# kkbwilldo/quantizations

Measured on AMD Instinct MI355X. Metric: decode tokens/sec Llama-3-8B NF4 bs=1; 4096×4096 GEMV GB/s vs HBM peak, higher is better.
Workload: dtype f16 activations x 4-bit NF4 weights (exact NF4 codes (fp32 as hi+lo fp16)), fp32 accumulate; 1 GPU; llama3-8b-nf4-dq-decode-bs1; layers=32, prompt_len=32, global_batch=1, stream_batch=1, decode=hipgraph, parallelism=single, projection_groups=64, layer_ops=229, compute_dtype=fp32, rmsnorm_in_grouped_gemv=True, decode_attention=qz_decode_attention, silu_in_gate_up_launch=True, residual_in_gemv_epilogue=True, lm_head=layer_ops.gemv_dense, lm_head_rows_split=False, attention=single GPU

## Files before the change

include/quantizations.h:

```cpp
#ifndef QUANTIZATIONS_H
#define QUANTIZATIONS_H

#ifdef __cplusplus
extern "C" {
#endif

#define QZ_DT_F16 0
#define QZ_DT_BF16 1
#define QZ_DT_F32 2

#define QZ_FP4 0
#define QZ_NF4 1
#define QZ_EXACT_CODES 0x100

#define QZ_OK 0
#define QZ_ERR_ARG (-1)
#define QZ_ERR_BLOCKSIZE (-2)
#define QZ_ERR_SHAPE (-3)
#define QZ_ERR_DTYPE (-4)


int cgemm_4bit_inference_naive_fp32(int m, int n, int k, float *A, unsigned char *B, float *absmax,
                                    float *datatype, float *out, int lda, int ldb, int ldc, int blocksize);

// ... 76 lines not shown
int qz_dequantize_blockwise_8bit(const float *code, const unsigned char *A, const float *absmax, long long n,
                                 int blocksize, const float *offset, float *out, void *stream);

int qz_dequantize_4bit(const unsigned char *A, long long n, int quant_type, int blocksize, const float *absmax,
                       const unsigned char *qabsmax, const float *absmax2, const float *code2, const float *offset,
                       int blocksize2, void *out, int out_dtype, void *stream);

int qz_bench_read_floor(const void *p, long long bytes, unsigned int *sink, void *stream);

int qz_bench_empty(unsigned int *sink, void *stream);

int qz_ipc_handle_size(void);
long long qz_exchange_bytes(int world, long long slot_bytes);
int qz_exchange_alloc(long long bytes, void **ptr);
int qz_exchange_free(void *ptr);
int qz_ipc_get_handle(const void *ptr, void *handle);
int qz_ipc_open_handle(const void *handle, void **ptr);
int qz_ipc_close_handle(void *ptr);
int qz_enable_peer_access(int peer_device);
int qz_allgather_oneshot(const void *src, int nbytes, void *dst, int rank, int world, void *const *peer_bufs,
                         void *own_buf, long long slot_bytes, unsigned int *epoch, unsigned int *status,
                         void *stream);
int qz_allgather_oneshot_mode(const void *src, int nbytes, void *dst, int rank, int world, void *const *peer_bufs,
                              void *own_buf, long long slot_bytes, unsigned int *epoch, unsigned int *status,
                              int mode, void *stream);


int qz_rmsnorm(const void *x, int dtype, long long rows, int K, long long ldx, const void *weight, float eps, void *y,
               long long ldy, void *stream);

int qz_add_rmsnorm(const void *x, const void *residual, int dtype, long long rows, int K, long long ldx,
                   const void *weight, float eps, void *sum, void *y, long long ldy, void *stream);

int qz_rope_qk(int dtype, int B, int S, int D, const void *q, int Hq, const long long *q_str, void *q_out,
               const long long *qo_str, const void *k, int Hk, const long long *k_str, void *k_out,
               const long long *ko_str, const void *cos, const void *sin, const long long *cs_str, void *stream);

int qz_silu_mul(const void *gate, const void *up, int dtype, long long n, void *y, void *stream);


int qz_decode_attention(int dtype, int B, int Hq, int Hkv, int D, int L, const void *q, long long q_row,
                        const void *k, long long k_row, const void *v, long long v_row, const void *cos,
                        const void *sin, long long cs_row, void *k_cache, void *v_cache, const void *mask,
                        long long mask_b, long long mask_j, long long *pos, unsigned int *arrive, void *out,
                        long long out_row, float *work, float scale, void *stream);

long long qz_greedy_step_work_bytes(int B, long long V);
int qz_greedy_step(const void *logits, int dtype, int B, long long V, long long row, long long *hist,
                   long long hist_row, long long hist_len, long long *pos, long long *tok, void *work, void *stream);
int qz_gemv_dense(int M, int K, const void *x, int dtype, const void *W, void *y, void *stream);
int qz_decode_mask(const long long *q_offset, int B, int L, void *mask, void *stream);
int qz_rope_table(int dtype, int B, int S, int D, const long long *pos, long long pos_b, long long pos_s,
                  const void *cos_table, const void *sin_table, long long T, const float *inv_freq, float scale,
                  void *cos, void *sin, void *stream);

int qz_gemv_4bit_pair_silu(const qz_gemv_segment *segs, int K, const void *x, int dtype, int quant_type,
                           int blocksize, int blocksize2, const float *lut, const void *norm_weight, float eps,
                           void *h, void *stream);

#define QZ_LORA_MAX_RANK 64
typedef struct qz_lora_shrink_segment {
  const void *A;
  const float *scaling;
  int r;
  int t_offset;
} qz_lora_shrink_segment;
int qz_lora_shrink(int nseg, const qz_lora_shrink_segment *segs, int K, const void *x, int dtype,
                   const void *norm_weight, float eps, float *t, void *stream);
int qz_gemv_4bit_lora(int M, int K, const void *x, int dtype, const unsigned char *B, int quant_type, int blocksize,
                      const float *absmax, const unsigned char *qabsmax, const float *absmax2, const float *code2,
                      const float *offset, int blocksize2, long long block_base, const float *lut, const void *bias,
                      const void *residual, const void *lora_B, int r, const float *t, void *y, void *stream);
typedef struct qz_lora_segment {
  const void *B;
  int r;
  int t_offset;
} qz_lora_segment;
int qz_gemv_4bit_grouped_lora(int nseg, const qz_gemv_segment *segs, const qz_lora_segment *lora, const float *t,
                              int K, const void *x, int dtype, int quant_type, int blocksize, int blocksize2,
                              const float *lut, const void *norm_weight, float eps, void *stream);

int qz_gemv_knobs(char *buf, int n);
int qz_gemv_set_knob(const char *name, int value);

int qz_version(void);

#ifdef __cplusplus
}
#endif

#endif
```

quantizations_amd/_lib.py:

```python
from __future__ import annotations

import ctypes
import os

import torch

HERE = os.path.dirname(os.path.abspath(__file__))
LIB_PATH = os.environ.get("QZ_LIB_PATH", os.path.join(HERE, "libquantizations.so"))

DT_F16, DT_BF16, DT_F32 = 0, 1, 2
FP4, NF4 = 0, 1
QUANT_TYPES = {"fp4": FP4, "nf4": NF4}
EXACT_CODES = 0x100

_STATUS = {
    -1: "invalid argument (null pointer or negative size)",
    -2: "unsupported blocksize",
    -3: "unsupported shape",
    -4: "unsupported dtype or quant type",
}

_p = ctypes.c_void_p
_i = ctypes.c_int
_ll = ctypes.c_longlong
_f = ctypes.c_float

GEMV_MAX_SEGMENTS = 4
QZ_ERR_SHAPE = -3


class GemvSegment(ctypes.Structure):
    _fields_ = [("M", ctypes.c_int), ("B", ctypes.c_void_p), ("absmax", ctypes.c_void_p),
                ("qabsmax", ctypes.c_void_p), ("absmax2", ctypes.c_void_p), ("code2", ctypes.c_void_p),
                ("offset", ctypes.c_void_p), ("block_base", ctypes.c_longlong), ("bias", ctypes.c_void_p),
                ("y", ctypes.c_void_p)]


class LoraSegment(ctypes.Structure):
    _fields_ = [("B", ctypes.c_void_p), ("r", ctypes.c_int), ("t_offset", ctypes.c_int)]


class LoraShrinkSegment(ctypes.Structure):
    _fields_ = [("A", ctypes.c_void_p), ("scaling", ctypes.c_void_p), ("r", ctypes.c_int),
                ("t_offset", ctypes.c_int)]


LORA_MAX_RANK = 64

SIGNATURES = {
    "cgemm_4bit_inference_naive_fp32": [_i, _i, _i, _p, _p, _p, _p, _p, _i, _i, _i, _i],
    "cquantize_blockwise_fp16_fp4": [_p, _p, _p, _p, _i, _i],
    "cdequantize_blockwise_fp16_fp4": [_p, _p, _p, _p, _i, _i],
    "cquantize_blockwise_fp32": [_p, _p, _p, _p, _i, _i],
    "cdequantize_blockwise_fp32": [_p, _p, _p, _p, _i, _i],
    "cgemm_4bit_inference_naive_fp32_stream": [_i, _i, _i, _p, _p, _p, _p, _p, _i, _i, _i, _i, _p],
    "cquantize_blockwise_fp16_fp4_stream": [_p, _p, _p, _p, _i, _i, _p],
    "cdequantize_blockwise_fp16_fp4_stream": [_p, _p, _p, _p, _i, _i, _p],
    "cquantize_blockwise_fp32_stream": [_p, _p, _p, _p, _i, _i, _p],
    "cdequantize_blockwise_fp32_stream": [_p, _p, _p, _p, _i, _i, _p],
    "qz_gemv_4bit": [_i, _i, _p, _i, _p, _i, _i, _p, _p, _p, _p, _p, _i, _ll, _p, _p, _p, _p],
    "qz_gemv_4bit_residual": [_i, _i, _p, _i, _p, _i, _i, _p, _p, _p, _p, _p, _i, _ll, _p, _p, _p, _p, _p],
    "qz_gemv_4bit_grouped": [_i, _p, _i, _p, _i, _i, _i, _i, _p, _p],
    "qz_gemv_4bit_grouped_rmsnorm": [_i, _p, _i, _p, _i, _i, _i, _i, _p, _p, _f, _p],
    "qz_gemv_4bit_pair_silu": [_p, _i, _p, _i, _i, _i, _i, _p, _p, _f, _p, _p],
    "qz_lora_shrink": [_i, _p, _i, _p, _i, _p, _f, _p, _p],
    "qz_gemv_4bit_lora": [_i, _i, _p, _i, _p, _i, _i, _p, _p, _p, _p, _p, _i, _ll, _p, _p, _p, _p, _i, _p, _p, _p],
    "qz_gemv_4bit_grouped_lora": [_i, _p, _p, _p, _i, _p, _i, _i, _i, _i, _p, _p, _f, _p],
    "qz_decode_attention": [_i, _i, _i, _i, _i, _i, _p, _ll, _p, _ll, _p, _ll, _p, _p, _ll, _p, _p, _p, _ll, _ll,
                            _p, _p, _p, _ll, _p, _f, _p],
    "qz_gemm_4bit": [_i, _i, _i, _p, _i, _i, _p, _i, _i, _p, _p, _p, _p, _p, _i, _p, _p, _i, _p, _ll, _p],
    "qz_gemm_4bit_workspace_size": [_i, _i, _i],
    "qz_gemm_16bit": [_i, _i, _i, _p, _i, _i, _p, _p, _p, _i, _p],
    "qz_gemm_16bit_ok": [_i, _i, _i, _p, _i, _p, _p, _i],
    "qz_gemm_4bit_grouped": [_i, _p, _i, _i, _p, _i, _i, _i, _i, _i, _p],
    "qz_quantize_4bit": [_p, _i, _ll, _i, _i, _p, _p, _p],
    "qz_absmax_mean_workspace": [_ll],
    "qz_absmax_mean": [_p, _ll, _p, _p, _p],
    "qz_quantize_blockwise_8bit": [_p, _p, _ll, _i, _p, _p, _p, _p],
    "qz_dequantize_blockwise_8bit": [_p, _p, _p, _ll, _i, _p, _p, _p],
    "qz_dequantize_4bit": [_p, _ll, _i, _i, _p, _p, _p, _p, _p, _i, _p, _i, _p],
    "qz_rmsnorm": [_p, _i, _ll, _i, _ll, _p, _f, _p, _ll, _p],
    "qz_rope_qk": [_i, _i, _i, _i, _p, _i, _p, _p, _p, _p, _i, _p, _p, _p, _p, _p, _p, _p],
    "qz_silu_mul": [_p, _p, _i, _ll, _p, _p],
    "qz_decode_mask": [_p, _i, _i, _p, _p],
    "qz_gemv_dense": [_i, _i, _p, _i, _p, _p, _p],
    "qz_greedy_step": [_p, _i, _i, _ll, _ll, _p, _ll, _ll, _p, _p, _p, _p],
    "qz_greedy_step_work_bytes": [_i, _ll],
    "qz_rope_table": [_i, _i, _i, _i, _p, _ll, _ll, _p, _p, _ll, _p, _f, _p, _p, _p],
    "qz_add_rmsnorm": [_p, _p, _i, _ll, _i, _ll, _p, _f, _p, _p, _ll, _p],
    "qz_bench_read_floor": [_p, _ll, _p, _p],
    "qz_bench_empty": [_p, _p],
    "qz_ipc_handle_size": [],
    "qz_exchange_bytes": [_i, _ll],
    "qz_exchange_alloc": [_ll, _p],
    "qz_exchange_free": [_p],
    "qz_ipc_get_handle": [_p, _p],
    "qz_ipc_open_handle": [_p, _p],
    "qz_ipc_close_handle": [_p],
    "qz_enable_peer_access": [_i],
    "qz_allgather_oneshot": [_p, _i, _p, _i, _i, _p, _p, _ll, _p, _p, _p],
    "qz_allgather_oneshot_mode": [_p, _i, _p, _i, _i, _p, _p, _ll, _p, _p, _i, _p],
    "qz_gemv_knobs": [_p, _i],
    "qz_gemv_set_knob": [ctypes.c_char_p, _i],
    "qz_version": [],
}
RESTYPES = {"qz_absmax_mean_workspace": _ll, "qz_gemm_4bit_workspace_size": _ll, "qz_exchange_bytes": _ll,
            "qz_greedy_step_work_bytes": _ll}


def _load():
    if not os.path.exists(LIB_PATH):
        raise ImportError(
            f"libquantizations.so not found at {LIB_PATH}: build it with "
            "`python -c 'import __graft_entry__ as g; g.build()'` (hipcc --offload-arch=gfx950)")
    lib = ctypes.CDLL(LIB_PATH)
    for name, args in SIGNATURES.items():
        fn = getattr(lib, name)
        fn.argtypes = args
        fn.restype = RESTYPES.get(name, _i)
    return lib


lib = _load()


class QuantizationsError(RuntimeError):
    pass


def check(rc: int, what: str) -> None:
    if rc != 0:
        msg = _STATUS.get(rc, f"HIP error {rc}")
        raise QuantizationsError(f"{what} failed: {msg}")


def dtype_code(dt: torch.dtype) -> int:
    if dt == torch.float16:
        return DT_F16
    if dt == torch.bfloat16:
        return DT_BF16
    if dt == torch.float32:
        return DT_F32
    raise NotImplementedError(f"dtype {dt} is not supported by the 4-bit kernels")


def stream_of(t: torch.Tensor) -> int:
    return torch.cuda.current_stream(t.device).cuda_stream


def ptr(t) -> int:
    return 0 if t is None else t.data_ptr()


def gemv_knobs() -> dict:
    import json
    buf = ctypes.create_string_buffer(512)
    n = lib.qz_gemv_knobs(buf, len(buf))
    return json.loads(buf.value.decode()) if 0 < n < len(buf) else {}


def set_gemv_knob(name: str, value: int) -> None:
    check(lib.qz_gemv_set_knob(name.encode(), int(value)), f"qz_gemv_set_knob({name})")
```

quantizations_amd/csrc/gemv.hip:

```cpp
#include "gemv_core.h"

namespace qz {

static int env_int(const char *name, int dflt) {
  const char *e = getenv(name);
  return e && *e ? atoi(e) : dflt;
}
static Knobs read_knobs() {
  Knobs k;
  k.wide8 = env_int("QZ_GEMV_WIDE8", 1) != 0;
  const int nr = env_int("QZ_GROUPED_NORM_R", 0);
  k.norm_r = (nr == 1 || nr == 2 || nr == 4) ? nr : 0;
  const int pr = env_int("QZ_PAIR_R", 0);
  k.pair_r = (pr == 2 || pr == 3 || pr == 4 || pr == 6 || pr == 8) ? pr : 0;
  k.pair_wt = env_int("QZ_PAIR_WT", 1) != 0;
  k.pair_ps = env_int("QZ_PAIR_PS", -1);
  k.pair_wk1 = env_int("QZ_PAIR_WK1", 2);
  return k;
}
static Knobs g_knobs = read_knobs();
Knobs &gemv_knobs() { return g_knobs; }
static int g_gemm16_sched = env_int("QZ_GEMM16_SCHED", 971);
int &gemm16_sched() { return g_gemm16_sched; }

template <bool DQ, int DT, int R, int WK, int NW, bool FS, bool CL, bool WT, bool TWO, int STAMP = 0>
__global__ __launch_bounds__(NW * 64) void k_gemv_4bit(GemvParams p) {
  gemv_body<DQ, DT, R, WK, NW, FS, CL, WT, false, false, TWO, false, STAMP>(p, blockIdx.x);
}

template <bool DQ, int DT, int R, int WK, bool FS, bool CL, bool NRM, bool TWO>
__global__ __launch_bounds__(256) void k_gemv_4bit_grouped(GemvGroup g) {
  const int b = blockIdx.x;
  int s = 0;
#pragma unroll
  for (int i = 1; i < kMaxSeg; ++i)
    if (i < g.nseg && b >= g.start[i]) s = i;
  s = __builtin_amdgcn_readfirstlane(s);
  const GemvParams seg = g.seg[s];
  const int start = g.start[s];
  gemv_body<DQ, DT, R, WK, 4, FS, CL, false, NRM, false, TWO, false>(seg, b - start);
}

template <bool DQ, int DT, int R, bool CL, bool NRM, bool TWO, bool PS = false, bool WT = false>
__global__ __launch_bounds__(256) void k_gemv_4bit_pair(GemvGroup g) {
  const int wave = __builtin_amdgcn_readfirstlane((int)threadIdx.x / kWave);
  const GemvParams seg = g.seg[wave >> 1];
  gemv_body<DQ, DT, R, 1, 4, true, CL, WT, NRM, true, TWO, PS>(seg, blockIdx.x, g.seg);
}

template <bool DQ, int DT>
__global__ __launch_bounds__(256) void k_gemv_4bit_generic(GemvParams p, int quant_type) {
  gemv_generic_body<DQ, DT>(p, quant_type);
}


template <bool DQ, int DT, bool FS, bool CL>
static void launch_vec(const GemvParams &p, int R, int WK, hipStream_t s) {
  const int RG = 4 / WK;
  const unsigned grid = (unsigned)((p.M + R * RG - 1) / (R * RG));
#define QZ_GV(RR, WW, TWO_) \
  hipLaunchKernelGGL((k_gemv_4bit<DQ, DT, RR, WW, 4, FS, CL, false, (WW == 1 && TWO_)>), dim3(grid), dim3(256), 0, s, p)
#define QZ_GV_RW(TWO_)                        \
  do {                                        \
    if (R == 4 && WK == 2) QZ_GV(4, 2, TWO_); \
    else if (R == 4) QZ_GV(4, 1, TWO_);       \
    else if (R == 2) QZ_GV(2, 1, TWO_);       \
    else if (WK == 1) QZ_GV(1, 1, TWO_);      \
    else if (WK == 2) QZ_GV(1, 2, TWO_);      \
    else QZ_GV(1, 4, TWO_);                   \
  } while (0)
  if constexpr (FS) {
    if (two_steps(p.K, WK, true)) { QZ_GV_RW(true); return; }
  }
  if constexpr (FS && CL && DT == QZ_DT_F16) {
    if (WK == 1 && (R == 2 || R == 4) && p.K >= 14336 && gemv_knobs().wide8) {
      const unsigned g8 = (unsigned)((p.M + R * 8 - 1) / (R * 8));
      if (R == 4) hipLaunchKernelGGL((k_gemv_4bit<DQ, DT, 4, 1, 8, FS, CL, true, false>), dim3(g8), dim3(512), 0, s, p);
      else hipLaunchKernelGGL((k_gemv_4bit<DQ, DT, 2, 1, 8, FS, CL, true, false>), dim3(g8), dim3(512), 0, s, p);
      return;
    }
  }
  QZ_GV_RW(false);
#undef QZ_GV_RW
#undef QZ_GV
}

template <bool DQ, bool FS, bool CL>
static int dispatch_dt(const GemvParams &p, int dtype, int R, int WK, hipStream_t s) {
  switch (dtype) {
    case QZ_DT_F16: launch_vec<DQ, QZ_DT_F16, FS, CL>(p, R, WK, s); return QZ_OK;
    case QZ_DT_BF16:
      if constexpr (!CL) { launch_vec<DQ, QZ_DT_BF16, FS, false>(p, R, WK, s); return QZ_OK; }
      break;
    case QZ_DT_F32:
      if constexpr (!CL) { launch_vec<DQ, QZ_DT_F32, FS, false>(p, R, WK, s); return QZ_OK; }
      break;
  }
// ... 97 lines not shown
      if (!full_steps(K, blocksize, blocksize2, dq, segs[i].block_base)) return QZ_ERR_SHAPE;
      g.seg[i].nw = nw;
      g.seg[i].eps = eps;
    }
  }
  if (!all_vec || total_m > INT32_MAX) {
    for (int i = 0; i < nseg; ++i) {
      const qz_gemv_segment &q = segs[i];
      const int rc = qz_gemv_4bit(q.M, K, x, dtype, q.B, quant_type, blocksize, q.absmax, q.qabsmax, q.absmax2,
                                  q.code2, q.offset, blocksize2, q.block_base, lut, q.bias, q.y, stream);
      if (rc != QZ_OK) return rc;
    }
    return QZ_OK;
  }
  int R, WK;
  choose_geometry((int)total_m, K, dtype, &R, &WK);
  if (nw && gemv_knobs().norm_r && WK == 1) R = gemv_knobs().norm_r;
  const int rows_per_block = R * (4 / WK);
  int blocks = 0;
  for (int i = 0; i < nseg; ++i) {
    set_tables(quant_type & ~QZ_EXACT_CODES, lut, cl, dtype, &g.seg[i]);
    g.start[i] = blocks;
    blocks += (g.seg[i].M + rows_per_block - 1) / rows_per_block;
  }
  for (int i = nseg; i < kMaxSeg; ++i) g.start[i] = blocks;
  g.total = blocks;
  if (nw && blocks > kNormMaxBlocks) return QZ_ERR_SHAPE;
  if (nw && WK != 1 && (long long)blocks * K > kNormSplitMaxValues) return QZ_ERR_SHAPE;
  bool all_fs = true;
  for (int i = 0; i < nseg; ++i) all_fs = all_fs && full_steps(K, blocksize, blocksize2, dq, segs[i].block_base);
  hipStream_t s = (hipStream_t)stream;
  const bool two = two_steps(K, WK, all_fs || nw);
  const size_t lds = nw ? (size_t)K * 2 : 0;
#define QZ_GR1(DQ_, DT_, RR, WW, FS_, CL_, NRM_)                                                            \
  do {                                                                                                    \
    if (FS_ && two && WW == 1)                                                                            \
      hipLaunchKernelGGL((k_gemv_4bit_grouped<DQ_, DT_, RR, WW, FS_, CL_, NRM_, (FS_ && WW == 1)>), dim3(blocks), \
                         dim3(256), lds, s, g);                                                           \
    else hipLaunchKernelGGL((k_gemv_4bit_grouped<DQ_, DT_, RR, WW, FS_, CL_, NRM_, false>), dim3(blocks),      \
                            dim3(256), lds, s, g);                                                        \
  } while (0)
#define QZ_GR_RW(DQ_, DT_, FS_, CL_, NRM_)                                                                  \
  do {                                                                                                    \
    if (R == 4 && WK == 2) QZ_GR1(DQ_, DT_, 4, 2, FS_, CL_, NRM_);                                        \
    else if (R == 4) QZ_GR1(DQ_, DT_, 4, 1, FS_, CL_, NRM_);                                              \
    else if (R == 2) QZ_GR1(DQ_, DT_, 2, 1, FS_, CL_, NRM_);                                              \
    else if (WK == 1) QZ_GR1(DQ_, DT_, 1, 1, FS_, CL_, NRM_);                                             \
    else if (WK == 2) QZ_GR1(DQ_, DT_, 1, 2, FS_, CL_, NRM_);                                             \
    else QZ_GR1(DQ_, DT_, 1, 4, FS_, CL_, NRM_);                                                          \
  } while (0)
#define QZ_GR_DT(DQ_, FS_)                                                                                  \
  do {                                                                                                    \
    if (dtype == QZ_DT_F16) { if (cl) QZ_GR_RW(DQ_, QZ_DT_F16, FS_, true, false); else QZ_GR_RW(DQ_, QZ_DT_F16, FS_, false, false); } \
    else if (dtype == QZ_DT_BF16) QZ_GR_RW(DQ_, QZ_DT_BF16, FS_, false, false);                         \
    else QZ_GR_RW(DQ_, QZ_DT_F32, FS_, false, false);                                                    \
  } while (0)
  if (nw) {
    if (dtype == QZ_DT_F16) {
      if (dq) { if (cl) QZ_GR_RW(true, QZ_DT_F16, true, true, true); else QZ_GR_RW(true, QZ_DT_F16, true, false, true); }
      else { if (cl) QZ_GR_RW(false, QZ_DT_F16, true, true, true); else QZ_GR_RW(false, QZ_DT_F16, true, false, true); }
    } else {
      if (dq) QZ_GR_RW(true, QZ_DT_BF16, true, false, true); else QZ_GR_RW(false, QZ_DT_BF16, true, false, true);
    }
  } else if (all_fs) { if (dq) QZ_GR_DT(true, true); else QZ_GR_DT(false, true); }
  else { if (dq) QZ_GR_DT(true, false); else QZ_GR_DT(false, false); }
#undef QZ_GR_DT
#undef QZ_GR_RW
#undef QZ_GR1
  QZ_LAUNCH_CHECK();
  return QZ_OK;
}

extern "C" int qz_gemv_4bit_grouped(int nseg, const qz_gemv_segment *segs, int K, const void *x, int dtype,
                                    int quant_type, int blocksize, int blocksize2, const float *lut, void *stream) {
  return gemv_grouped_impl(nseg, segs, K, x, dtype, quant_type, blocksize, blocksize2, lut, nullptr, 0.0f, stream);
}

extern "C" int qz_gemv_4bit_grouped_rmsnorm(int nseg, const qz_gemv_segment *segs, int K, const void *x, int dtype,
                                            int quant_type, int blocksize, int blocksize2, const float *lut,
                                            const void *norm_weight, float eps, void *stream) {
  if (!norm_weight || !x) return QZ_ERR_ARG;
  return gemv_grouped_impl(nseg, segs, K, x, dtype, quant_type, blocksize, blocksize2, lut, norm_weight, eps, stream);
}

template <bool DQ, int DT, int R, bool CL, bool NRM>
static void launch_pair_wt(unsigned grid, size_t lds, hipStream_t s, const GemvGroup &g, bool two) {
  if constexpr (CL && NRM && DT == QZ_DT_F16 && (R == 2 || R == 4)) {
    if (two) hipLaunchKernelGGL((k_gemv_4bit_pair<DQ, DT, R, CL, NRM, true, true, true>), dim3(grid), dim3(256), lds, s, g);
    else hipLaunchKernelGGL((k_gemv_4bit_pair<DQ, DT, R, CL, NRM, false, true, true>), dim3(grid), dim3(256), lds, s, g);
  }
}

template <bool DQ, int DT, int R, bool CL, bool NRM>
static void launch_pair_ps_loop(unsigned grid, int blocks, size_t lds, hipStream_t s, const GemvGroup &g) {
  if constexpr (NRM)
    hipLaunchKernelGGL((k_gemv_4bit_pair<DQ, DT, R, CL, NRM, false, true>), dim3(grid), dim3(256), lds, s, g);
  else
    hipLaunchKernelGGL((k_gemv_4bit_pair<DQ, DT, R, CL, NRM, false>), dim3(blocks), dim3(256), lds, s, g);
}

extern "C" int qz_gemv_4bit_pair_silu(const qz_gemv_segment *segs, int K, const void *x, int dtype, int quant_type,
                                      int blocksize, int blocksize2, const float *lut, const void *norm_weight,
                                      float eps, void *h, void *stream) {
  if (!segs || !h || !x) return QZ_ERR_ARG;
  if (segs[0].M != segs[1].M) return QZ_ERR_SHAPE;
  if (dtype != QZ_DT_F16 && dtype != QZ_DT_BF16) return QZ_ERR_SHAPE;
  GemvGroup g;
  g.nseg = 2;
  const bool cl = exact_codes(quant_type, lut) && dtype == QZ_DT_F16;
  const bool dq = segs[0].qabsmax != nullptr;
  for (int i = 0; i < 2; ++i) {
    const qz_gemv_segment &q = segs[i];
    bool v;
    const int st = make_params(q.M, K, x, dtype, q.B, quant_type, blocksize, q.absmax, q.qabsmax, q.absmax2, q.code2,
                               q.offset, blocksize2, q.block_base, lut, q.bias, h, &g.seg[i], &v);
    if (st != QZ_OK) return st;
    if ((q.qabsmax != nullptr) != dq || !v || !full_steps(K, blocksize, blocksize2, dq, q.block_base))
      return QZ_ERR_SHAPE;
    set_tables(quant_type & ~QZ_EXACT_CODES, lut, cl, dtype, &g.seg[i]);
    g.seg[i].nw = norm_weight;
    g.seg[i].eps = eps;
  }
  const int M = segs[0].M;
  if (M == 0) return QZ_OK;
  if (norm_weight && (K % 8 != 0 || K > 16384 || ((uintptr_t)x | (uintptr_t)norm_weight) % 16 != 0))
    return QZ_ERR_SHAPE;
  int R, WK;
  choose_geometry(2 * M, K, dtype, &R, &WK);
  if (WK != 1) {
    const int wk1 = gemv_knobs().pair_wk1;
    if (wk1 == 0 || (norm_weight && wk1 != 2)) return QZ_ERR_SHAPE;
    WK = 1;
  }
  if (gemv_knobs().pair_r) R = gemv_knobs().pair_r;
  const int blocks = (M + 2 * R - 1) / (2 * R);
  if (norm_weight && blocks > kNormMaxBlocks) return QZ_ERR_SHAPE;
  for (int i = 2; i < kMaxSeg; ++i) g.start[i] = 0;
  hipStream_t s = (hipStream_t)stream;
  const size_t lds = norm_weight ? (size_t)K * 2 : 0;
  const bool two = two_steps(K, 1, true);
  const int cus = device_cus();
  const size_t img = norm_weight ? (size_t)K * 2 : 0;
  const int per_cu_wt = (int)std::min<size_t>(3, kLdsPerCU / (2 * kTabDwords * 4 + img + 4096));
  const int per_cu = (int)std::min<size_t>(3, kLdsPerCU / (kTabDwords * 4 + img + 4096));
  const bool wt_ok = cl && norm_weight && (R == 2 || R == 4) && blocks >= 3 * 2 * cus && per_cu_wt >= 2 &&
                     gemv_knobs().pair_wt;
  int pgrid_i = 0;
  if (gemv_knobs().pair_ps >= 0) {
    const int ps = gemv_knobs().pair_ps;
    pgrid_i = ps <= 0 ? 0 : ps <= 8 ? cus * ps : ps;
  } else if (norm_weight) {
    pgrid_i = (wt_ok ? 2 : per_cu) * cus;
  }
  const unsigned pgrid = (unsigned)max(pgrid_i, 1);
  const bool persist = pgrid_i > 0 && pgrid_i < blocks;
  const bool pair_wt = persist && wt_ok;
#define QZ_PS(DQ_, DT_, RR, CL_, NRM_)                                                                               \
  do {                                                                                                              \
    if (pair_wt) launch_pair_wt<DQ_, DT_, RR, CL_, NRM_>(pgrid, lds, s, g, two);                                        \
    else if (persist && two) hipLaunchKernelGGL((k_gemv_4bit_pair<DQ_, DT_, RR, CL_, NRM_, true, true>), dim3(pgrid), \
                                                dim3(256), lds, s, g);                                              \
    else if (persist) launch_pair_ps_loop<DQ_, DT_, RR, CL_, NRM_>(pgrid, blocks, lds, s, g);                      \
    else if (two) hipLaunchKernelGGL((k_gemv_4bit_pair<DQ_, DT_, RR, CL_, NRM_, true>), dim3(blocks), dim3(256),    \
                                     lds, s, g);                                                                    \
    else hipLaunchKernelGGL((k_gemv_4bit_pair<DQ_, DT_, RR, CL_, NRM_, false>), dim3(blocks), dim3(256), lds, s, g); \
  } while (0)
#define QZ_PS_R(DQ_, DT_, CL_, NRM_)                  \
  do {                                                \
    if (R == 4) QZ_PS(DQ_, DT_, 4, CL_, NRM_);        \
    else if (R == 8) QZ_PS(DQ_, DT_, 8, CL_, NRM_);   \
    else if (R == 6) QZ_PS(DQ_, DT_, 6, CL_, NRM_);   \
    else if (R == 3) QZ_PS(DQ_, DT_, 3, CL_, NRM_);   \
    else if (R == 1) QZ_PS(DQ_, DT_, 1, CL_, NRM_);   \
    else QZ_PS(DQ_, DT_, 2, CL_, NRM_);               \
  } while (0)
#define QZ_PS_N(DQ_, DT_, CL_)                                                         \
  do {                                                                                 \
    if (norm_weight) QZ_PS_R(DQ_, DT_, CL_, true); else QZ_PS_R(DQ_, DT_, CL_, false); \
  } while (0)
  if (dtype == QZ_DT_F16) {
    if (dq) { if (cl) QZ_PS_N(true, QZ_DT_F16, true); else QZ_PS_N(true, QZ_DT_F16, false); }
    else { if (cl) QZ_PS_N(false, QZ_DT_F16, true); else QZ_PS_N(false, QZ_DT_F16, false); }
  } else {
    if (dq) QZ_PS_N(true, QZ_DT_BF16, false); else QZ_PS_N(false, QZ_DT_BF16, false);
  }
#undef QZ_PS_N
#undef QZ_PS_R
#undef QZ_PS
  QZ_LAUNCH_CHECK();
  return QZ_OK;
}

extern "C" int qz_gemv_knobs(char *buf, int n) {
  char tmp[320];
  const int len = snprintf(tmp, sizeof(tmp),
                           "{\"QZ_GEMV_WIDE8\": %d, \"QZ_GROUPED_NORM_R\": %d, \"QZ_PAIR_R\": %d, \"QZ_PAIR_WT\": %d, "
                           "\"QZ_PAIR_PS\": %d, \"QZ_PAIR_WK1\": %d, \"QZ_GEMM16_SCHED\": %d, \"cus\": %d}",
                           gemv_knobs().wide8, gemv_knobs().norm_r, gemv_knobs().pair_r, gemv_knobs().pair_wt,
                           gemv_knobs().pair_ps, gemv_knobs().pair_wk1, gemm16_sched(), device_cus());
  if (buf && n > len) memcpy(buf, tmp, (size_t)len + 1);
  return len;
}

extern "C" int qz_gemv_set_knob(const char *name, int value) {
  if (!name) return QZ_ERR_ARG;
  Knobs &k = gemv_knobs();
  if (!strcmp(name, "QZ_GEMV_WIDE8")) k.wide8 = value != 0;
  else if (!strcmp(name, "QZ_GROUPED_NORM_R")) k.norm_r = (value == 1 || value == 2 || value == 4) ? value : 0;
  else if (!strcmp(name, "QZ_PAIR_R")) k.pair_r = (value == 2 || value == 3 || value == 4 || value == 6 || value == 8) ? value : 0;
  else if (!strcmp(name, "QZ_PAIR_WT")) k.pair_wt = value != 0;
  else if (!strcmp(name, "QZ_PAIR_PS")) k.pair_ps = value;
  else if (!strcmp(name, "QZ_PAIR_WK1")) k.pair_wk1 = value;
  else if (!strcmp(name, "QZ_GEMM16_SCHED")) gemm16_sched() = value;
  else return QZ_ERR_ARG;
  return QZ_OK;
}
```

quantizations_amd/csrc/gemv_core.h:

```cpp
#pragma once
#include "common.h"

#include <atomic>
#include <cstdio>
#include <cstdlib>
#include <cstring>

namespace qz {

constexpr int kTabCopies = 32;
constexpr int kTabDwords = 256 * kTabCopies;
constexpr int kTabCopiesCL = 16;

constexpr uint16_t f16_bits_rne_c(float f) {
  const uint32_t u = __builtin_bit_cast(uint32_t, f);
  const uint32_t sign = (u >> 16) & 0x8000u, au = u & 0x7FFFFFFFu;
  if (au == 0) return (uint16_t)sign;
  const uint32_t e = (au >> 23) - 127u + 15u, m = au & 0x7FFFFFu;
  uint32_t h = (e << 10) | (m >> 13);
  const uint32_t rem = m & 0x1FFFu;
  if (rem > 0x1000u || (rem == 0x1000u && (h & 1u))) h += 1u;
  return (uint16_t)(sign | h);
}
struct ByteTable {
// ... 12 lines not shown
                                0.7229568362236023f, 1.0f};
constexpr ByteTable make_nf4_table() {
  uint16_t c[16] = {};
  for (int i = 0; i < 16; ++i) c[i] = f16_bits_rne_c(kNF4Host[i]);
  return make_byte_table(c);
}
constexpr uint16_t kFP4x12Bits[16] = {0x0000, 0x2C00, 0x4800, 0x4A00, 0x4400, 0x4600, 0x4000, 0x4200,
                                      0x8000, 0xAC00, 0xC800, 0xCA00, 0xC400, 0xC600, 0xC000, 0xC200};
constexpr int kNF4ExactShift = 14;
constexpr float f16_value_c(uint16_t h) {
  const float sgn = (h & 0x8000u) ? -1.0f : 1.0f;
  const int e = (h >> 10) & 31;
  if (e == 0) return sgn * 0.0f;
  float v = 1.0f + (float)(h & 0x3FFu) / 1024.0f;
  for (int i = 15; i < e; ++i) v *= 2.0f;
  for (int i = e; i < 15; ++i) v *= 0.5f;
  return sgn * v;
}
constexpr ByteTable make_nf4_exact_table() {
  uint16_t hi[16] = {}, lo[16] = {};
  for (int i = 0; i < 16; ++i) {
    const float c = kNF4Host[i] * (float)(1 << kNF4ExactShift);
    hi[i] = f16_bits_rne_c(c);
    lo[i] = f16_bits_rne_c(c - f16_value_c(hi[i]));
  }
  ByteTable t{};
  for (int e = 0; e < 256; ++e) {
    const uint32_t h = (uint32_t)hi[e >> 4] | ((uint32_t)hi[e & 15] << 16);
    const uint32_t l = (uint32_t)lo[e >> 4] | ((uint32_t)lo[e & 15] << 16);
    t.v[4 * e + 0] = h; t.v[4 * e + 1] = l; t.v[4 * e + 2] = h; t.v[4 * e + 3] = l;
  }
  return t;
}
constexpr uint16_t bf16_bits_rne_c(float f) {
  const uint32_t u = __builtin_bit_cast(uint32_t, f);
  return (uint16_t)((u + 0x7FFFu + ((u >> 16) & 1u)) >> 16);
}
constexpr float bf16_value_c(uint16_t b) { return __builtin_bit_cast(float, (uint32_t)b << 16); }
constexpr ByteTable make_bf16_table(const float (&c)[16]) {
  uint16_t hi[16] = {}, lo[16] = {};
  for (int i = 0; i < 16; ++i) {
    hi[i] = bf16_bits_rne_c(c[i]);
    lo[i] = bf16_bits_rne_c(c[i] - bf16_value_c(hi[i]));
  }
  ByteTable t{};
  for (int e = 0; e < 256; ++e) {
    const uint32_t h = (uint32_t)hi[e >> 4] | ((uint32_t)hi[e & 15] << 16);
    const uint32_t l = (uint32_t)lo[e >> 4] | ((uint32_t)lo[e & 15] << 16);
    t.v[4 * e + 0] = h; t.v[4 * e + 1] = l; t.v[4 * e + 2] = h; t.v[4 * e + 3] = l;
  }
  return t;
}
constexpr float kFP4x12Host[16] = {0.0f, 0.0625f, 8.0f, 12.0f, 4.0f, 6.0f, 2.0f, 3.0f,
                                   -0.0f, -0.0625f, -8.0f, -12.0f, -4.0f, -6.0f, -2.0f, -3.0f};
constexpr ByteTable make_f32_table(const float (&c)[16]) {
  ByteTable t{};
  for (int e = 0; e < 256; ++e) {
    const uint32_t a = __builtin_bit_cast(uint32_t, c[e >> 4]), b = __builtin_bit_cast(uint32_t, c[e & 15]);
    t.v[4 * e + 0] = a; t.v[4 * e + 1] = b; t.v[4 * e + 2] = a; t.v[4 * e + 3] = b;
  }
  return t;
}
static __device__ const ByteTable g_byte_tab_nf4 = make_nf4_table();
static __device__ const ByteTable g_byte_tab_nf4x = make_nf4_exact_table();
static __device__ const ByteTable g_byte_tab_fp4 = make_byte_table(kFP4x12Bits);
static __device__ const ByteTable g_byte_tab_nf4_bf = make_bf16_table(kNF4Host);
static __device__ const ByteTable g_byte_tab_fp4_bf = make_bf16_table(kFP4x12Host);
static __device__ const ByteTable g_byte_tab_nf4_f32 = make_f32_table(kNF4Host);
static __device__ const ByteTable g_byte_tab_fp4_f32 = make_f32_table(kFP4x12Host);
static_assert(bf16_bits_rne_c(0.07958029955625534f) == 0x3DA3, "bf16 RNE of an NF4 code");
static_assert(f16_bits_rne_c(0.07958029955625534f) == 0x2D18, "fp16 RNE of an NF4 code");

typedef uint32_t u32x4 __attribute__((ext_vector_type(4)));
typedef uint32_t u32x2 __attribute__((ext_vector_type(2)));
typedef __bf16 bf16x2_t __attribute__((ext_vector_type(2)));

template <int DT> __device__ __forceinline__ float round_store(float v) {
  if constexpr (DT == QZ_DT_F16) return __half2float(__ushort_as_half(f32_to_f16_bits(v)));
  else if constexpr (DT == QZ_DT_BF16) return __bfloat162float(__float2bfloat16(v));
  else return v;
}
template <int DT> __device__ __forceinline__ float add_res(float o, const void *res, long long row) {
  return res ? __fadd_rn(load_f32<DT>(res, row), round_store<DT>(o)) : o;
}

template <int DT> __device__ __forceinline__ uint32_t pack16(float a, float b) {
  if constexpr (DT == QZ_DT_F16) {
    return (uint32_t)f32_to_f16_bits(a) | ((uint32_t)f32_to_f16_bits(b) << 16);
  } else {
    return (uint32_t)__builtin_bit_cast(uint16_t, __float2bfloat16(a)) |
           ((uint32_t)__builtin_bit_cast(uint16_t, __float2bfloat16(b)) << 16);
  }
}

struct GemvParams {
  const unsigned char *B;
  const void *x;
  ScaleSrc sc;
  const void *bias;
  void *y;
  const float *lut;
  long long block_base;
  int M, K;
  int bs_log2, bs2_log2;
  float out_scale;
  int tabsel;
  const void *nw;
  float eps;
  const void *res;
};

struct LoraOp {
  const void *B;
  const float *t;
  int r;
};

__device__ __forceinline__ float dot2(uint32_t a, uint32_t b, float c) {
  return __builtin_amdgcn_fdot2(__builtin_bit_cast(h2_t, a), __builtin_bit_cast(h2_t, b), c, false);
}

template <typename T> __device__ __forceinline__ T keep_s(T v) {
  asm volatile("" : "+s"(v));
  return v;
}
template <typename T> __device__ __forceinline__ T *keep_sp(T *v) {
  typedef __attribute__((address_space(1))) T *gptr;
  gptr g = (gptr)v;
  asm volatile("" : "+s"(g));
  return (T *)g;
}

#ifdef QZ_STAMPS
__device__ unsigned long long *g_qz_stamp;
#define QZ_STAMP_DECL unsigned long long qz_st_[6] = {0, 0, 0, 0, 0, 0}
#define QZ_STAMP(k)                                                                  \
  do {                                                                               \
    if constexpr ((STAMP & 3) != 0 && ((STAMP & 3) == 1 || (k) == 0 || (k) == 4)) {  \
      __builtin_amdgcn_sched_barrier(0);                                             \
      asm volatile("s_memrealtime %0\n\ts_waitcnt lgkmcnt(0)" : "=s"(qz_st_[k])::"memory"); \
      __builtin_amdgcn_sched_barrier(0);                                             \
    }                                                                                \
  } while (0)
#define QZ_STAMP_FLUSH(wave_id)                                                      \
  do {                                                                               \
    if constexpr ((STAMP & 3) != 0) {                                                \
      uint32_t xcc, hw;                                                              \
      asm volatile("s_getreg_b32 %0, hwreg(HW_REG_XCC_ID)" : "=s"(xcc));             \
      asm volatile("s_getreg_b32 %0, hwreg(HW_REG_HW_ID)" : "=s"(hw));               \
      qz_st_[5] = ((unsigned long long)xcc << 32) | hw;                              \
      if ((threadIdx.x & 63) == 0) {                                                 \
        if constexpr ((STAMP & 3) == 2) {                                            \
          g_qz_stamp[(size_t)(wave_id) * 8 + 0] = qz_st_[0];                         \
          g_qz_stamp[(size_t)(wave_id) * 8 + 4] = qz_st_[4];                         \
        } else {                                                                     \
          for (int k_ = 0; k_ < 6; ++k_) g_qz_stamp[(size_t)(wave_id) * 8 + k_] = qz_st_[k_]; \
        }                                                                            \
      }                                                                              \
    }                                                                                \
  } while (0)
#else
#define QZ_STAMP_DECL
#define QZ_STAMP(k) do {} while (0)
#define QZ_STAMP_FLUSH(wave_id) do {} while (0)
#endif

// ... 271 lines not shown
__device__ __forceinline__ uint32_t norm_x_off(uint32_t chunk) {
  const uint32_t s = chunk >> 8, l = (chunk >> 2) & 63u, i = chunk & 3u;
  return (s << 12) + (l << 6) + ((i ^ ((l >> 2) & 3u)) << 4);
}

constexpr int kMaxSeg = 4;
struct GemvGroup {
  GemvParams seg[kMaxSeg];
  int start[kMaxSeg];
  int nseg;
  int total;
};
struct LoraGroup {
  LoraOp seg[kMaxSeg];
};

template <bool DQ, int DT, int R, int WK, int NW, bool FS, bool CL, bool WT, bool NRM, bool PAIR, bool TWO, bool PS,
          int STAMP = 0, bool LORA = false>
__device__ __forceinline__ void gemv_body(const GemvParams &p_in, const int block, const GemvParams *pair = nullptr,
                                          const LoraOp *lora = nullptr) {
  static_assert(!LORA || (!PAIR && DT != QZ_DT_F32), "adapter operand: single / grouped launches, 16-bit activations");
  static_assert(!NRM || (NW == 4 && FS && DT != QZ_DT_F32), "fused pre-norm: 4 waves, full steps, 16-bit activations");
  static_assert(!PAIR || (NW == 4 && WK == 1 && DT != QZ_DT_F32), "pair: 4 waves, WK = 1, 16-bit activations");
  static_assert(!PS || (PAIR && FS), "persistent form: pair launches, full steps");
  static_assert(!TWO || (FS && WK == 1), "two-step form: full steps, whole rows per wave");
  static_assert(!CL || DT == QZ_DT_F16, "exact codes are the fp16-activation table");
  static_assert(NW * 64 >= 256, "one byte-table entry per thread");
  constexpr int kPieces = WT ? 16 : kTabCopies / 4;
  QZ_STAMP_DECL;
  QZ_STAMP(0);
  const GemvParams p = load_params(p_in);
  constexpr int RG = NW / WK;
  constexpr bool kBF = DT == QZ_DT_BF16;
  constexpr bool kF32 = DT == QZ_DT_F32;
  constexpr bool kWide = CL || kBF || kF32;
  __shared__ float s_code2[PAIR ? 2 : 1][DQ ? 256 : 1];
  __shared__ float s_part[NW][R];
  __shared__ float s_part2[PS ? 2 : 1][NW][R];
  __shared__ __attribute__((aligned(16))) uint32_t s_tab[(WT ? 2 : 1) * kTabDwords];
  extern __shared__ __attribute__((aligned(16))) unsigned char s_x[];

  const int lane = threadIdx.x & (kWave - 1);
  const int wave = __builtin_amdgcn_readfirstlane(threadIdx.x / kWave);
  const int wk = wave % WK;
  const int rg = wave / WK;
  int row0 = PAIR ? (block * 2 + (wave & 1)) * R : (block * RG + rg) * R;
  const int cb = PAIR ? (wave >> 1) : 0;
  const int row_bytes = p.K >> 1;
  const int nsteps = (row_bytes + 1023) >> 10;

  float c2 = 0.0f, c2b = 0.0f, offset = 0.0f;
  if constexpr (DQ) {
    if constexpr (PAIR) {
      c2 = keep_sp(pair[0].sc.code2)[threadIdx.x];
      c2b = keep_sp(pair[1].sc.code2)[threadIdx.x];
    } else if (NW * 64 == 256 || threadIdx.x < 256) {
      c2 = p.sc.code2[threadIdx.x & 255];
    }
    offset = *p.sc.offset;
  }
  u32x4 tab_entry = {0u, 0u, 0u, 0u};
  if (!p.lut && threadIdx.x < 256) {
    const ByteTable *bt = kF32 ? (p.tabsel ? &g_byte_tab_fp4_f32 : &g_byte_tab_nf4_f32)
                          : kBF ? (p.tabsel ? &g_byte_tab_fp4_bf : &g_byte_tab_nf4_bf)
                                : (CL ? &g_byte_tab_nf4x : (p.tabsel ? &g_byte_tab_fp4 : &g_byte_tab_nf4));
    tab_entry = reinterpret_cast<const u32x4 *>(bt->v)[threadIdx.x];
  }
  constexpr int kNChunks = NRM ? 8 : 1;
  constexpr int kNHeld = NRM ? 2 : 1;
  u32x4 nx[kNChunks], nwh[kNHeld];
  const int n_nchunk = p.K >> 3;
  if constexpr (NRM) {
#pragma unroll
    for (int i = 0; i < kNChunks; ++i) {
      const int c = (int)threadIdx.x + 256 * i;
      if (c < n_nchunk) nx[i] = reinterpret_cast<const u32x4 *>(p.x)[c];
    }
#pragma unroll
    for (int i = 0; i < kNHeld; ++i) {
      const int c = (int)threadIdx.x + 256 * i;
      if (c < n_nchunk) nwh[i] = reinterpret_cast<const u32x4 *>(p.nw)[c];
    }
    __builtin_amdgcn_sched_barrier(0);
  }
  typedef StepLoads<DQ, DT, R, NRM, FS> Loads;
  Loads cur, other;
  int s = wk;
  cur.issue(p, row0, s < nsteps ? s : 0, lane, row_bytes);
  float lo_b[LORA ? R : 1], lo_t = 0.0f;
  bool lo_on = false;
  if constexpr (LORA) {
    const int lr = keep_s(lora->r);
    const char *lB = reinterpret_cast<const char *>(keep_sp(lora->B));
    const float *lt = keep_sp(lora->t);
    lo_on = lane < lr && wk == 0;
    const int j = lo_on ? lane : 0;
    lo_t = lt[j];
#pragma unroll
    for (int r = 0; r < R; ++r) {
      const size_t row = (size_t)min(row0 + r, p.M - 1);
      lo_b[r] = load_f32<DT>(lB + row * (size_t)lr * 2u, j);
    }
  }
  const bool have = s < nsteps;
  const int n_my = have ? (nsteps - wk + WK - 1) / WK : 0;
  if constexpr (DQ) {
    if (NW * 64 == 256 || threadIdx.x < 256) s_code2[0][threadIdx.x & 255] = c2;
    if constexpr (PAIR) s_code2[PAIR ? 1 : 0][threadIdx.x] = c2b;
  }
  __shared__ float s_nss[NRM ? 4 : 1];
  if constexpr (NRM) {
    float ss = 0.0f;
#pragma unroll
    for (int i = 0; i < kNChunks; ++i)
      if ((int)threadIdx.x + 256 * i < n_nchunk) ss = norm_chunk_ss<DT>(nx[i], ss);
    ss = norm_wave_sum(ss);
    if (lane == 0) s_nss[wave] = ss;
  }
  float out_scale = p.out_scale;
  if constexpr (kF32) {
    if (p.lut) {
      out_scale = 1.0f;
      build_byte_table_f32<NW * 64, kPieces>(s_tab, p.lut);
    } else if (threadIdx.x < 256) {
      store_byte_table_entry<kPieces>(s_tab, tab_entry);
    }
  } else if constexpr (kBF) {
    if (p.lut) {
      out_scale = 1.0f;
      build_byte_table_bf16<NW * 64, kPieces>(s_tab, p.lut);
    } else if (threadIdx.x < 256) {
      store_byte_table_entry<kPieces>(s_tab, tab_entry);
    }
  } else if constexpr (CL) {
    if (p.lut) {
      const int S = lut_shift(p.lut);
      out_scale = ldexpf(1.0f, -S);
      build_byte_table_exact<NW * 64, kPieces>(s_tab, p.lut, S);
    } else if (threadIdx.x < 256 && (STAMP & 48) == 0) {
      store_byte_table_entry<kPieces>(s_tab, tab_entry);
    }
  } else if (threadIdx.x < 256) {
    store_byte_table_entry<kPieces>(s_tab, tab_entry);
  }
  if constexpr ((STAMP & 32) == 0) __syncthreads();
  if constexpr (NRM) {
    const float tot = __fadd_rn(__fadd_rn(s_nss[0], s_nss[1]), __fadd_rn(s_nss[2], s_nss[3]));
    const float rs = rsqrtf(__fadd_rn(__fmul_rn(tot, 1.0f / (float)p.K), p.eps));
#pragma unroll
    for (int i = 0; i < kNChunks; ++i) {
      const int c = (int)threadIdx.x + 256 * i;
      if (c < n_nchunk) {
        const u32x4 xv = i < kNHeld ? nx[i] : reinterpret_cast<const u32x4 *>(p.x)[c];
        const u32x4 wv = i < kNHeld ? nwh[i < kNHeld ? i : 0] : reinterpret_cast<const u32x4 *>(p.nw)[c];
        *reinterpret_cast<u32x4 *>(s_x + norm_x_off((uint32_t)c)) = norm_chunk_apply<DT>(xv, wv, rs);
      }
    }
    __syncthreads();
  }
  QZ_STAMP(1);
  const uint32_t jb = WT ? (kWide ? (uint32_t)(lane & 31) << 3 : (uint32_t)lane << 2)
                        : (kWide ? (uint32_t)(lane & (kTabCopiesCL - 1)) << 3 : (uint32_t)(lane & 31) << 2);

  float acc[R];
#pragma unroll
  for (int r = 0; r < R; ++r) acc[r] = 0.0f;
// ... 81 lines not shown
        } else {
          consume(cur);
        }
      }
      const int nb = blk + (int)gridDim.x;
      if (nb >= nblocks) {
        pair_out(blk, it & 1);
        break;
      }
      const int nrow0 = (nb * 2 + (wave & 1)) * R;
      cur.issue(p, nrow0, s, lane, row_bytes);
      __builtin_amdgcn_sched_barrier(0);
      pair_out(blk, it & 1);
#pragma unroll
      for (int r = 0; r < R; ++r) acc[r] = 0.0f;
      blk = nb;
      row0 = nrow0;
    }
    return;
  } else if constexpr (TWO) {
    other.issue(p, row0, s + WK, lane, row_bytes);
    __builtin_amdgcn_sched_barrier(0);
    consume(cur);
    QZ_STAMP(2);
    consume(other);
  } else if (have) {
    const int n = n_my;
    int j = 0;
    for (; j + 2 < n; j += 2) {
      other.issue(p, row0, s + WK, lane, row_bytes);
      __builtin_amdgcn_sched_barrier(0);
      consume(cur);
      cur.issue(p, row0, s + 2 * WK, lane, row_bytes);
      __builtin_amdgcn_sched_barrier(0);
      consume(other);
      s += 2 * WK;
    }
    if (n - j == 2) {
      other.issue(p, row0, s + WK, lane, row_bytes);
      __builtin_amdgcn_sched_barrier(0);
      consume(cur);
      QZ_STAMP(2);
      consume(other);
    } else {
      consume(cur);
    }
  }

  if constexpr (LORA) {
    const float inv = __fdiv_rn(1.0f, out_scale);
#pragma unroll
    for (int r = 0; r < R; ++r) acc[r] = lo_on ? fmaf(__fmul_rn(lo_b[r], lo_t), inv, acc[r]) : acc[r];
  }
  QZ_STAMP(3);
  if constexpr (PAIR) {
    float v[R];
#pragma unroll
    for (int r = 0; r < R; ++r) v[r] = wave_sum_last(acc[r]);
    if (lane == kWave - 1) {
#pragma unroll
      for (int r = 0; r < R; ++r) {
        float o = v[r] * out_scale;
        if (p.bias) o += load_f32<DT>(p.bias, min(row0 + r, p.M - 1));
        s_part[wave][r] = o;
      }
    }
    __syncthreads();
    if ((int)threadIdx.x < 2 * R) {
      const int g2 = threadIdx.x / R, r = threadIdx.x % R;
      const int row = (block * 2 + g2) * R + r;
      if (row < p.M) {
        const float gv = round_store<DT>(s_part[g2][r]), uv = round_store<DT>(s_part[2 + g2][r]);
        const float a = round_store<DT>(__fdiv_rn(gv, __fadd_rn(1.0f, expf(-gv))));
        store_f32<DT>(keep_sp(pair[0].y), row, __fmul_rn(a, uv));
      }
    }
    return;
  }
  if constexpr (WK == 1) {
    float v[R];
#pragma unroll
    for (int r = 0; r < R; ++r) v[r] = wave_sum_last(acc[r]);
    if (lane == kWave - 1) {
      constexpr bool kPack = DT != QZ_DT_F32 && R % 2 == 0;
      const bool pack = kPack && row0 + R <= p.M && (reinterpret_cast<uintptr_t>(p.y) & 3u) == 0;
      if (pack) {
#pragma unroll
        for (int r = 0; r < R; r += 2) {
          float o0 = v[r] * out_scale, o1 = v[r + 1] * out_scale;
          if (p.bias) {
            o0 += load_f32<DT>(p.bias, row0 + r);
            o1 += load_f32<DT>(p.bias, row0 + r + 1);
          }
          o0 = add_res<DT>(o0, p.res, row0 + r);
          o1 = add_res<DT>(o1, p.res, row0 + r + 1);
          reinterpret_cast<uint32_t *>(p.y)[(row0 + r) >> 1] = pack16<DT>(o0, o1);
        }
      } else {
#pragma unroll
        for (int r = 0; r < R; ++r) {
          const int row = row0 + r;
          if (row < p.M) {
            float o = v[r] * out_scale;
            if (p.bias) o += load_f32<DT>(p.bias, row);
            o = add_res<DT>(o, p.res, row);
            store_f32<DT>(p.y, row, o);
          }
        }
      }
    }
    QZ_STAMP(4);
    QZ_STAMP_FLUSH(block * NW + wave);
    return;
  }
#pragma unroll
  for (int r = 0; r < R; ++r) {
    const float v = wave_sum_last(acc[r]);
    if (lane == kWave - 1) s_part[wave][r] = v;
  }
  __syncthreads();
  if ((int)threadIdx.x < RG * R) {
    const int g = threadIdx.x / R, r = threadIdx.x % R;
    const int row = (block * RG + g) * R + r;
    if (row < p.M) {
      float v = 0.0f;
#pragma unroll
      for (int k = 0; k < WK; ++k) v += s_part[g * WK + k][r];
      v *= out_scale;
      if (p.bias) v += load_f32<DT>(p.bias, row);
      store_f32<DT>(p.y, row, add_res<DT>(v, p.res, row));
    }
  }
}

template <bool DQ, int DT, bool LORA = false>
__device__ __forceinline__ void gemv_generic_body(const GemvParams &p, int quant_type, const LoraOp *lora = nullptr) {
  __shared__ float s_lut[16];
  if (threadIdx.x < 16) s_lut[threadIdx.x] = p.lut ? p.lut[threadIdx.x] : 0.0f;
  __syncthreads();
  const int lane = threadIdx.x & (kWave - 1);
  const int row = blockIdx.x * 4 + threadIdx.x / kWave;
  if (row >= p.M) return;
  const float offset = DQ ? *p.sc.offset : 0.0f;
  float acc = 0.0f;
  for (int k = lane; k < p.K; k += kWave) {
    const long long e = (long long)row * p.K + k;
    const uint32_t byte = p.B[e >> 1];
    const uint32_t nib = (e & 1) ? (byte & 0xFu) : (byte >> 4);
    const long long b = p.block_base + (e >> p.bs_log2);
    float am;
    if constexpr (DQ) am = __fadd_rn(__fmul_rn(p.sc.code2[p.sc.qabsmax[b]], p.sc.absmax2[b >> p.bs2_log2]), offset);
    else am = p.sc.absmax[b];
    float c;
    if (p.lut) c = s_lut[nib];
    else if (quant_type == QZ_NF4) c = kNF4[nib];
    else c = (nib & 8u ? -1.0f : 1.0f) * dequant_fp4_tree(nib & 7u, 1.0f);
    acc = fmaf(load_f32<DT>(p.x, k), __fmul_rn(c, am), acc);
  }
  if constexpr (LORA) {
    if (lane < lora->r) acc = fmaf(load_f32<DT>(lora->B, (long long)row * lora->r + lane), lora->t[lane], acc);
  }
  acc = wave_sum_last(acc);
  if (lane == kWave - 1) {
    if (p.bias) acc += load_f32<DT>(p.bias, row);
    store_f32<DT>(p.y, row, add_res<DT>(acc, p.res, row));
  }
}


struct Knobs {
  int wide8;
  int norm_r;
  int pair_r;
  int pair_wt;
  int pair_ps;
  int pair_wk1;
};
constexpr int kNormMaxBlocks = 4096;
constexpr long long kNormSplitMaxValues = 1LL << 23;
constexpr size_t kLdsPerCU = 160 * 1024;
Knobs &gemv_knobs();

static int ilog2(long long v) {
  int l = 0;
  while ((1LL << l) < v) ++l;
  return (1LL << l) == v ? l : -1;
}

// ... 74 lines not shown
```

Measured before the change: 553.2 tokens/s.

## Prefetch residual/bias in GEMV prologue and base pair persistence on geometry

For non-pair, single-split, 4-wave GEMV kernels, the residual and bias values are now loaded into registers before the main loop instead of in the epilogue, which hides their load latency behind weight streaming. The pair (gate/up + SiLU) launcher now decides whether the wide-table persistent path applies using the default-R block count and the actual persistent grid size rather than a fixed 2×CUs. It also allows R=1 as a pair knob and records the last pair launch geometry for inspection. Holding the extra per-row values in registers may raise register pressure, and loads are issued for all lanes rather than only the storing lane.

```diff
diff --git a/include/quantizations.h b/include/quantizations.h
--- a/include/quantizations.h
+++ b/include/quantizations.h
@@ -182,6 +182,7 @@
 
 int qz_gemv_knobs(char *buf, int n);
 int qz_gemv_set_knob(const char *name, int value);
+int qz_gemv_pair_last_geometry(int *out);
 
 int qz_version(void);
 
diff --git a/quantizations_amd/_lib.py b/quantizations_amd/_lib.py
--- a/quantizations_amd/_lib.py
+++ b/quantizations_amd/_lib.py
@@ -102,6 +102,7 @@
     "qz_allgather_oneshot_mode": [_p, _i, _p, _i, _i, _p, _p, _ll, _p, _p, _i, _p],
     "qz_gemv_knobs": [_p, _i],
     "qz_gemv_set_knob": [ctypes.c_char_p, _i],
+    "qz_gemv_pair_last_geometry": [_p],
     "qz_version": [],
 }
 RESTYPES = {"qz_absmax_mean_workspace": _ll, "qz_gemm_4bit_workspace_size": _ll, "qz_exchange_bytes": _ll,
@@ -159,5 +160,11 @@
     return json.loads(buf.value.decode()) if 0 < n < len(buf) else {}
 
 
+def pair_last_geometry() -> dict:
+    out = (ctypes.c_int * 4)()
+    check(lib.qz_gemv_pair_last_geometry(ctypes.cast(out, ctypes.c_void_p)), "qz_gemv_pair_last_geometry")
+    return {"R": out[0], "grid": out[1], "blocks": out[2], "wide_table": bool(out[3])}
+
+
 def set_gemv_knob(name: str, value: int) -> None:
     check(lib.qz_gemv_set_knob(name.encode(), int(value)), f"qz_gemv_set_knob({name})")
diff --git a/quantizations_amd/csrc/gemv.hip b/quantizations_amd/csrc/gemv.hip
--- a/quantizations_amd/csrc/gemv.hip
+++ b/quantizations_amd/csrc/gemv.hip
@@ -6,13 +6,14 @@
   const char *e = getenv(name);
   return e && *e ? atoi(e) : dflt;
 }
+static bool pair_r_ok(int r) { return r == 1 || r == 2 || r == 3 || r == 4 || r == 6 || r == 8; }
 static Knobs read_knobs() {
   Knobs k;
   k.wide8 = env_int("QZ_GEMV_WIDE8", 1) != 0;
   const int nr = env_int("QZ_GROUPED_NORM_R", 0);
   k.norm_r = (nr == 1 || nr == 2 || nr == 4) ? nr : 0;
   const int pr = env_int("QZ_PAIR_R", 0);
-  k.pair_r = (pr == 2 || pr == 3 || pr == 4 || pr == 6 || pr == 8) ? pr : 0;
+  k.pair_r = pair_r_ok(pr) ? pr : 0;
   k.pair_wt = env_int("QZ_PAIR_WT", 1) != 0;
   k.pair_ps = env_int("QZ_PAIR_PS", -1);
   k.pair_wk1 = env_int("QZ_PAIR_WK1", 2);
@@ -276,6 +277,8 @@
   if (!norm_weight || !x) return QZ_ERR_ARG;
   return gemv_grouped_impl(nseg, segs, K, x, dtype, quant_type, blocksize, blocksize2, lut, norm_weight, eps, stream);
 }
+
+static int g_pair_last[4] = {0, 0, 0, 0};
 
 template <bool DQ, int DT, int R, bool CL, bool NRM>
 static void launch_pair_wt(unsigned grid, size_t lds, hipStream_t s, const GemvGroup &g, bool two) {
@@ -326,6 +329,7 @@
     if (wk1 == 0 || (norm_weight && wk1 != 2)) return QZ_ERR_SHAPE;
     WK = 1;
   }
+  const int blocks_geom = (M + 2 * R - 1) / (2 * R);
   if (gemv_knobs().pair_r) R = gemv_knobs().pair_r;
   const int blocks = (M + 2 * R - 1) / (2 * R);
   if (norm_weight && blocks > kNormMaxBlocks) return QZ_ERR_SHAPE;
@@ -337,18 +341,21 @@
   const size_t img = norm_weight ? (size_t)K * 2 : 0;
   const int per_cu_wt = (int)std::min<size_t>(3, kLdsPerCU / (2 * kTabDwords * 4 + img + 4096));
   const int per_cu = (int)std::min<size_t>(3, kLdsPerCU / (kTabDwords * 4 + img + 4096));
-  const bool wt_ok = cl && norm_weight && (R == 2 || R == 4) && blocks >= 3 * 2 * cus && per_cu_wt >= 2 &&
-                     gemv_knobs().pair_wt;
+  const int ps_knob = gemv_knobs().pair_ps;
+  const int knob_grid = ps_knob <= 0 ? 0 : ps_knob <= 8 ? cus * ps_knob : ps_knob;
+  const int wt_grid = ps_knob >= 0 ? knob_grid : 2 * cus;
+  const bool wt_ok = cl && norm_weight && (R == 2 || R == 4) && blocks_geom >= 3 * wt_grid &&
+                     per_cu_wt >= 2 && gemv_knobs().pair_wt;
   int pgrid_i = 0;
-  if (gemv_knobs().pair_ps >= 0) {
-    const int ps = gemv_knobs().pair_ps;
-    pgrid_i = ps <= 0 ? 0 : ps <= 8 ? cus * ps : ps;
-  } else if (norm_weight) {
-    pgrid_i = (wt_ok ? 2 : per_cu) * cus;
-  }
+  if (ps_knob >= 0) pgrid_i = knob_grid;
+  else if (norm_weight) pgrid_i = (wt_ok ? 2 : per_cu) * cus;
   const unsigned pgrid = (unsigned)max(pgrid_i, 1);
   const bool persist = pgrid_i > 0 && pgrid_i < blocks;
   const bool pair_wt = persist && wt_ok;
+  g_pair_last[0] = R;
+  g_pair_last[1] = persist ? pgrid_i : blocks;
+  g_pair_last[2] = blocks;
+  g_pair_last[3] = pair_wt;
 #define QZ_PS(DQ_, DT_, RR, CL_, NRM_)                                                                               \
   do {                                                                                                              \
     if (pair_wt) launch_pair_wt<DQ_, DT_, RR, CL_, NRM_>(pgrid, lds, s, g, two);                                        \
@@ -385,6 +392,12 @@
   return QZ_OK;
 }
 
+extern "C" int qz_gemv_pair_last_geometry(int *out) {
+  if (!out) return QZ_ERR_ARG;
+  memcpy(out, g_pair_last, sizeof(g_pair_last));
+  return QZ_OK;
+}
+
 extern "C" int qz_gemv_knobs(char *buf, int n) {
   char tmp[320];
   const int len = snprintf(tmp, sizeof(tmp),
@@ -401,7 +414,7 @@
   Knobs &k = gemv_knobs();
   if (!strcmp(name, "QZ_GEMV_WIDE8")) k.wide8 = value != 0;
   else if (!strcmp(name, "QZ_GROUPED_NORM_R")) k.norm_r = (value == 1 || value == 2 || value == 4) ? value : 0;
-  else if (!strcmp(name, "QZ_PAIR_R")) k.pair_r = (value == 2 || value == 3 || value == 4 || value == 6 || value == 8) ? value : 0;
+  else if (!strcmp(name, "QZ_PAIR_R")) k.pair_r = pair_r_ok(value) ? value : 0;
   else if (!strcmp(name, "QZ_PAIR_WT")) k.pair_wt = value != 0;
   else if (!strcmp(name, "QZ_PAIR_PS")) k.pair_ps = value;
   else if (!strcmp(name, "QZ_PAIR_WK1")) k.pair_wk1 = value;
diff --git a/quantizations_amd/csrc/gemv_core.h b/quantizations_amd/csrc/gemv_core.h
--- a/quantizations_amd/csrc/gemv_core.h
+++ b/quantizations_amd/csrc/gemv_core.h
@@ -118,6 +118,9 @@
 }
 template <int DT> __device__ __forceinline__ float add_res(float o, const void *res, long long row) {
   return res ? __fadd_rn(load_f32<DT>(res, row), round_store<DT>(o)) : o;
+}
+template <int DT> __device__ __forceinline__ float add_res_value(float o, bool has_res, float res) {
+  return has_res ? __fadd_rn(res, round_store<DT>(o)) : o;
 }
 
 template <int DT> __device__ __forceinline__ uint32_t pack16(float a, float b) {
@@ -555,6 +558,20 @@
       if (c < n_nchunk) nwh[i] = reinterpret_cast<const u32x4 *>(p.nw)[c];
     }
     __builtin_amdgcn_sched_barrier(0);
+  }
+  constexpr bool kEarlyEp = !PAIR && WK == 1 && NW == 4;
+  float ep_res[R], ep_bias[R];
+  if constexpr (kEarlyEp) {
+#pragma unroll
+    for (int r = 0; r < R; ++r) ep_res[r] = ep_bias[r] = 0.0f;
+    if (p.res) {
+#pragma unroll
+      for (int r = 0; r < R; ++r) ep_res[r] = load_f32<DT>(p.res, min(row0 + r, p.M - 1));
+    }
+    if (p.bias) {
+#pragma unroll
+      for (int r = 0; r < R; ++r) ep_bias[r] = load_f32<DT>(p.bias, min(row0 + r, p.M - 1));
+    }
   }
   typedef StepLoads<DQ, DT, R, NRM, FS> Loads;
   Loads cur, other;
@@ -802,6 +819,14 @@
 #pragma unroll
     for (int r = 0; r < R; ++r) v[r] = wave_sum_last(acc[r]);
     if (lane == kWave - 1) {
+      auto bias_of = [&](int r, int row) {
+        if constexpr (kEarlyEp) return ep_bias[r];
+        else return load_f32<DT>(p.bias, row);
+      };
+      auto with_res = [&](float o, int r, int row) {
+        if constexpr (kEarlyEp) return add_res_value<DT>(o, p.res != nullptr, ep_res[r]);
+        else return add_res<DT>(o, p.res, row);
+      };
       constexpr bool kPack = DT != QZ_DT_F32 && R % 2 == 0;
       const bool pack = kPack && row0 + R <= p.M && (reinterpret_cast<uintptr_t>(p.y) & 3u) == 0;
       if (pack) {
@@ -809,11 +834,11 @@
         for (int r = 0; r < R; r += 2) {
           float o0 = v[r] * out_scale, o1 = v[r + 1] * out_scale;
           if (p.bias) {
-            o0 += load_f32<DT>(p.bias, row0 + r);
-            o1 += load_f32<DT>(p.bias, row0 + r + 1);
+            o0 += bias_of(r, row0 + r);
+            o1 += bias_of(r + 1, row0 + r + 1);
           }
-          o0 = add_res<DT>(o0, p.res, row0 + r);
-          o1 = add_res<DT>(o1, p.res, row0 + r + 1);
+          o0 = with_res(o0, r, row0 + r);
+          o1 = with_res(o1, r + 1, row0 + r + 1);
           reinterpret_cast<uint32_t *>(p.y)[(row0 + r) >> 1] = pack16<DT>(o0, o1);
         }
       } else {
@@ -822,8 +847,8 @@
           const int row = row0 + r;
           if (row < p.M) {
             float o = v[r] * out_scale;
-            if (p.bias) o += load_f32<DT>(p.bias, row);
-            o = add_res<DT>(o, p.res, row);
+            if (p.bias) o += bias_of(r, row);
+            o = with_res(o, r, row);
             store_f32<DT>(p.y, row, o);
           }
         }
```

Result: no change. 553.2 tokens/s, median of 2 (-0.0%).
